# Dizzy-cell/HOUV

Hardware: AMD Instinct MI355X
Metric: registration pairs/sec (2048-pt partial pairs) (higher is better)
Workload: dtype f32; 1 GPU; HOUV solve_model, 2048x2048-pt pairs, batch 256/GPU, K=64 restarts x 200 Adam iterations + retry stages (BASELINE configs[1]); pairs_per_gpu=256, points=2048, kernel=64, iters=200, icp_refine=False, parallelism=dp1 (pair shards, one RCCL all-gather of [steps*P,12] per rank)

## Files before the change

houv_amd/csrc/houv_math.h:

```cpp
#pragma once
#include <math.h>

#if defined(__HIPCC__)
#define HOUV_HD __host__ __device__
#else
#define HOUV_HD
#endif

namespace houv {

constexpr float kPiF = 3.14159274101257324f;

enum TransMode { kTransHouv = 0, kTransSolve = 1 };

HOUV_HD inline float tsqrt(float x) { return sqrtf(x); }
HOUV_HD inline double tsqrt(double x) { return sqrt(x); }

struct Pose {
  float R[9];
  float T[3];
  float u[3], inv_vnorm, sin_t, cos_t, chat[3], inv_cnorm, sigma, a, s;
};

HOUV_HD inline void pose_forward(const float p[8], int angle_base, int trans_mode, Pose& o) {
// ... 34 lines not shown
      AtM[i * 3 + j] = A[0 * 3 + i] * M[0 * 3 + j] + A[1 * 3 + i] * M[1 * 3 + j] + A[2 * 3 + i] * M[2 * 3 + j];
    }
  float dth = 0.f;
  for (int i = 0; i < 9; ++i) dth += M[i] * (f.cos_t * A[i] + f.sin_t * AA[i]);
  g[3] = dth * cosf(f.a * kPiF) * kPiF * kPiF / 8.0f;
  float Qm[9];
  const float omc = 1.0f - f.cos_t;
  for (int i = 0; i < 9; ++i) Qm[i] = f.sin_t * M[i] + omc * (MAt[i] + AtM[i]);
  const float du0 = Qm[7] - Qm[5], du1 = Qm[2] - Qm[6], du2 = Qm[3] - Qm[1];
  const float dot_u = ux * du0 + uy * du1 + uz * du2;
  g[0] = (du0 - ux * dot_u) * f.inv_vnorm;
  g[1] = (du1 - uy * dot_u) * f.inv_vnorm;
  g[2] = (du2 - uz * dot_u) * f.inv_vnorm;
  const float dot_c = f.chat[0] * gT[0] + f.chat[1] * gT[1] + f.chat[2] * gT[2];
  g[4] = f.sigma * (gT[0] - f.chat[0] * dot_c) * f.inv_cnorm;
  g[5] = f.sigma * (gT[1] - f.chat[1] * dot_c) * f.inv_cnorm;
  g[6] = f.sigma * (gT[2] - f.chat[2] * dot_c) * f.inv_cnorm;
  const float dsig = (trans_mode == kTransHouv) ? (cosf(f.s * kPiF) * kPiF * 0.125f) : (cosf(f.s * kPiF) * kPiF);
  g[7] = dot_c * dsig;
}

struct AdamScalars {
  double step_size, bc2_sqrt;
};
HOUV_HD inline AdamScalars adam_scalars(int step, double lr, double b1, double b2) {
  const double bc1 = 1.0 - pow(b1, (double)step);
  const double bc2 = 1.0 - pow(b2, (double)step);
  return AdamScalars{lr / bc1, sqrt(bc2)};
}
template <typename T>
HOUV_HD inline void adam_step(T& p, T& m, T& v, T g, const AdamScalars& sc, double b1, double b2, double eps) {
  m = m + (g - m) * (T)(1.0 - b1);
  v = v * (T)b2 + ((T)(1.0 - b2) * g) * g;
  const T denom = tsqrt(v) / (T)sc.bc2_sqrt + (T)eps;
  p = p - (T)sc.step_size * (m / denom);
}
template <typename T>
HOUV_HD inline void adam_step(T& p, T& m, T& v, T g, int step, double lr, double b1, double b2, double eps) {
  adam_step<T>(p, m, v, g, adam_scalars(step, lr, b1, b2), b1, b2, eps);
}

constexpr int kAccN = 13;
constexpr int kAccStride = 16;

struct TailLoss {
  float score, loss;
  float cd[4][2];
  float g[8];
};

template <int NMET>
HOUV_HD inline void solve_tail_loss(const float* acc, int acc_stride, const Pose& f, int k_full, int k_view, float loss_scale,
                                    int trans_mode, TailLoss& r) {
  float val[NMET];
  int pick[NMET];
  float gT[3] = {0.f, 0.f, 0.f}, Mm[9] = {0.f, 0.f, 0.f, 0.f, 0.f, 0.f, 0.f, 0.f, 0.f};
  bool bad = false;
#pragma unroll
  for (int m = 0; m < 4; ++m) r.cd[m][0] = r.cd[m][1] = 0.f;
#pragma unroll
  for (int m = 0; m < NMET; ++m) {
    const float kk = (float)((m == 0) ? k_full : k_view);
    r.cd[m][0] = acc[(m * 2 + 0) * acc_stride] / kk;
    r.cd[m][1] = acc[(m * 2 + 1) * acc_stride] / kk;
    pick[m] = (r.cd[m][0] <= r.cd[m][1]) ? 0 : 1;
    val[m] = r.cd[m][pick[m]];
    if (r.cd[m][0] != r.cd[m][0] || r.cd[m][1] != r.cd[m][1]) { val[m] = NAN; bad = true; }
    const float w = ((m == 0) ? 6.0f : 1.0f) * loss_scale / kk;
    const float* ac = acc + (m * 2 + pick[m]) * acc_stride;
#pragma unroll
    for (int i = 0; i < 3; ++i) gT[i] += w * ac[1 + i];
#pragma unroll
    for (int i = 0; i < 9; ++i) Mm[i] += w * ac[4 + i];
  }
  r.score = val[0];
  r.loss = val[0] * 6.0f;
  if constexpr (NMET == 4) r.loss = r.loss + (val[1] + val[2] + val[3]);
  if (bad) {
#pragma unroll
    for (int i = 0; i < 3; ++i) gT[i] = NAN;
#pragma unroll
    for (int i = 0; i < 9; ++i) Mm[i] = NAN;
  }
  pose_backward(f, trans_mode, gT, Mm, r.g);
}

HOUV_HD inline void solve_tail_step(const float g[8], double* state, int f64_params, AdamScalars asc, double beta1, double beta2,
                                    double eps, int angle_base, int trans_mode, Pose& next) {
  if (f64_params) {
    for (int k = 0; k < 8; ++k)
      adam_step<double>(state[k], state[8 + k], state[16 + k], (double)g[k], asc, beta1, beta2, eps);
  } else {
    for (int k = 0; k < 8; ++k) {
      float pp = (float)state[k], mm = (float)state[8 + k], vv = (float)state[16 + k];
      adam_step<float>(pp, mm, vv, g[k], asc, beta1, beta2, eps);
      state[k] = pp; state[8 + k] = mm; state[16 + k] = vv;
    }
  }
  float p[8];
#pragma unroll
  for (int k = 0; k < 8; ++k) p[k] = (float)state[k];
  pose_forward(p, angle_base, trans_mode, next);
}

constexpr int kTermAnchorFloats = 20;
constexpr float kTermRel = 1e-3f;
constexpr float kTermAbs = 1e-6f;
constexpr float kTermMoveErr = 1e-6f;

template <int NMET>
HOUV_HD inline unsigned term_masks(const float* anchor, const float* R, const float* T, float radius) {
  float fr = 0.f, ft = 0.f, tn = 0.f, ta = 0.f;
#pragma unroll
  for (int i = 0; i < 9; ++i) {
    const float d = R[i] - anchor[8 + i];
    fr += d * d;
  }
#pragma unroll
  for (int i = 0; i < 3; ++i) {
    const float d = T[i] - anchor[17 + i];
    ft += d * d;
    tn += T[i] * T[i];
    ta += anchor[17 + i] * anchor[17 + i];
  }
  const float delta2 = 2.0f * (sqrtf(fr) * radius + sqrtf(ft));
  const float abs_margin = kTermAbs + kTermMoveErr * (2.0f * radius + sqrtf(tn) + sqrtf(ta));
  unsigned need = ((1u << NMET) - 1u) * 0x11u;
#pragma unroll
  for (int m = 0; m < NMET; ++m) {
    const float c0 = anchor[2 * m], c1 = anchor[2 * m + 1];
    const float slack = delta2 + kTermRel * (fabsf(c0) + fabsf(c1) + delta2) + abs_margin;
    const unsigned drop1 = (c0 + slack < c1) ? (0x10u << m) : 0u;
    const unsigned drop0 = (c1 + slack < c0) ? (1u << m) : 0u;
    need &= ~(drop0 | drop1);
  }
  return need;
}

constexpr float kTermDefectMax = 1e-3f;
constexpr float kTermDefectErr = 1e-6f;

HOUV_HD inline float term_rot_defect(const float* M) {
  float s = 0.f;
#pragma unroll
  for (int i = 0; i < 3; ++i)
#pragma unroll
    for (int j = i; j < 3; ++j) {
      const float g = M[i] * M[j] + M[3 + i] * M[3 + j] + M[6 + i] * M[6 + j] - ((i == j) ? 1.0f : 0.0f);
      s += ((i == j) ? 1.0f : 2.0f) * g * g;
    }
  return sqrtf(s) + kTermDefectErr;
}

HOUV_HD inline void term_travel(const float* Rz, const float* Tz, const float* R, const float* T, float def_now, float radius,
                                float& d, float& tz) {
  float fr = 0.f, ft = 0.f, ta = 0.f;
#pragma unroll
  for (int i = 0; i < 9; ++i) {
    const float e = R[i] - Rz[i];
    fr += e * e;
  }
#pragma unroll
  for (int i = 0; i < 3; ++i) {
    const float e = T[i] - Tz[i];
    ft += e * e;
    ta += Tz[i] * Tz[i];
  }
  const float fro = sqrtf(fr), defect = def_now + term_rot_defect(Rz);
  const float tight = fro * 0.70710683f + 2.0f * defect;
  const bool ok = (fr <= 2.0f) & (defect <= kTermDefectMax) & (tight < fro);
  d = (ok ? tight : fro) * radius + sqrtf(ft);
  tz = sqrtf(ta);
}

template <int NMET>
HOUV_HD inline unsigned term_anchor_masks(const float* cd, const float* fresh, const float* stale, int stride,
                                          unsigned stale_bits, const float* R, const float* T, float radius_in) {
  const float radius = fabsf(radius_in);
  const float def_now = term_rot_defect(R);
  const float tn = sqrtf(T[0] * T[0] + T[1] * T[1] + T[2] * T[2]);
  float d_f, t_f;
  term_travel(fresh, fresh + 9, R, T, def_now, radius, d_f, t_f);
  unsigned need = ((1u << NMET) - 1u) * 0x11u;
#pragma unroll
  for (int m = 0; m < NMET; ++m) {
    float Rs[9], Ts[3], d_s, t_s;
#pragma unroll
    for (int i = 0; i < 9; ++i) Rs[i] = stale[(m * 12 + i) * stride];
#pragma unroll
    for (int i = 0; i < 3; ++i) Ts[i] = stale[(m * 12 + 9 + i) * stride];
    term_travel(Rs, Ts, R, T, def_now, radius, d_s, t_s);
    const bool s0 = (stale_bits >> m) & 1u, s1 = (stale_bits >> (4 + m)) & 1u;
    const float d0 = s0 ? d_s : d_f, d1 = s1 ? d_s : d_f;
    const float t0 = s0 ? t_s : t_f, t1 = s1 ? t_s : t_f;
    const float c0 = cd[2 * m], c1 = cd[2 * m + 1];
    const float dd = d0 + d1;
    const float slack = dd + kTermRel * (fabsf(c0) + fabsf(c1) + dd) + kTermAbs +
                        kTermMoveErr * (2.0f * radius + tn + 0.5f * (t0 + t1));
    const unsigned drop1 = (c0 + slack < c1) ? (0x10u << m) : 0u;
    const unsigned drop0 = (c1 + slack < c0) ? (1u << m) : 0u;
    need &= ~(drop0 | drop1);
  }
  return need;
}

constexpr int kWalkSets[] = {6, 11, 12, 13, 15};
constexpr int kNumWalkSets = (int)(sizeof(kWalkSets) / sizeof(kWalkSets[0]));
constexpr int walk_step_cost(unsigned mset) {
  const int k0 = (int)(mset & 1u), k1 = (int)((mset >> 1) & 1u), k2 = (int)((mset >> 2) & 1u), k3 = (int)((mset >> 3) & 1u);
  return 16 * (2 * (k0 + k1 + k2 + ((k0 | k3) ? 1 : 0)) + 2 * k1 + (k0 + k1 + k2 + k3)) + 5 * (k0 + k1 + k2 + k3);
}
constexpr bool walk_instantiated(unsigned mset) {
  for (int i = 0; i < kNumWalkSets; ++i)
    if ((unsigned)kWalkSets[i] == mset) return true;
  return false;
}
constexpr unsigned walk_variant(unsigned need) {
  unsigned best = 15u;
  for (int i = 0; i < kNumWalkSets; ++i) {
    const unsigned s = (unsigned)kWalkSets[i];
    if ((s & need) == need && walk_step_cost(s) < walk_step_cost(best)) best = s;
  }
  return best;
}
static_assert(walk_instantiated(15u) && walk_variant(15u) == 15u && walk_step_cost(15u) == 16 * 14 + 20, "today's code is a variant");
constexpr unsigned long long walk_variant_table() {
  unsigned long long t = 0ull;
  for (unsigned n = 0; n < 16u; ++n) t |= (unsigned long long)walk_variant(n) << (4 * n);
  return t;
}

HOUV_HD inline float box_med3(float a, float b, float c) {
#if defined(__HIP_DEVICE_COMPILE__)
  return __builtin_amdgcn_fmed3f(a, b, c);
#else
  if (a != a || b != b || c != c) return fminf(fminf(a, b), c);
  return fmaxf(fminf(a, b), fminf(fmaxf(a, b), c));
#endif
}

template <int NMET>
HOUV_HD inline bool box_within_bounds(float dx, float dy, float dz, const float* b, unsigned mset) {
  if constexpr (NMET == 4) {
    const float xx = dx * dx, yy = dy * dy;
    const float s3 = __builtin_fmaf(dy, dy, xx), s1 = __builtin_fmaf(dz, dz, yy), s2 = __builtin_fmaf(dz, dz, xx);
    const float s0 = __builtin_fmaf(dz, dz, s3);
    bool in = false;
    if (mset & 1u) in |= s0 <= b[0];
    if (mset & 2u) in |= s1 <= b[1];
    if (mset & 4u) in |= s2 <= b[2];
    if (mset & 8u) in |= s3 <= b[3];
    return in;
  } else {
    return __builtin_fmaf(dz, dz, __builtin_fmaf(dy, dy, dx * dx)) <= b[0];
  }
}

template <int NMET>
HOUV_HD inline bool box_test_query(const float* q, const float* lo, const float* hi, const float* ub, unsigned mset) {
  return box_within_bounds<NMET>(q[0] - box_med3(q[0], lo[0], hi[0]), q[1] - box_med3(q[1], lo[1], hi[1]),
                                 q[2] - box_med3(q[2], lo[2], hi[2]), ub, mset);
}

HOUV_HD inline float box_group_gap(float glo, float ghi, float lo, float hi) {
  return fmaxf(fmaxf(fminf(lo, hi) - ghi, glo - fmaxf(lo, hi)), 0.0f);
}

template <int NMET>
HOUV_HD inline bool box_test_group(const float* glo, const float* ghi, const float* lo, const float* hi, const float* gub,
                                   unsigned mset) {
  return box_within_bounds<NMET>(box_group_gap(glo[0], ghi[0], lo[0], hi[0]), box_group_gap(glo[1], ghi[1], lo[1], hi[1]),
                                 box_group_gap(glo[2], ghi[2], lo[2], hi[2]), gub, mset);
}

template <typename T>
HOUV_HD inline void svd3x3(const T H[9], T U[9], T S[3], T V[9]) {
  T B[9];
  for (int i = 0; i < 9; ++i) { B[i] = H[i]; V[i] = (i % 4 == 0) ? (T)1 : (T)0; }
  const int P[3] = {0, 0, 1}, Qi[3] = {1, 2, 2};
  for (int sweep = 0; sweep < 12; ++sweep) {
    T off = 0;
    for (int r = 0; r < 3; ++r) {
      const int p = P[r], q = Qi[r];
      const T a = B[0 * 3 + p] * B[0 * 3 + p] + B[1 * 3 + p] * B[1 * 3 + p] + B[2 * 3 + p] * B[2 * 3 + p];
      const T b = B[0 * 3 + q] * B[0 * 3 + q] + B[1 * 3 + q] * B[1 * 3 + q] + B[2 * 3 + q] * B[2 * 3 + q];
      const T g = B[0 * 3 + p] * B[0 * 3 + q] + B[1 * 3 + p] * B[1 * 3 + q] + B[2 * 3 + p] * B[2 * 3 + q];
      const T eps2 = sizeof(T) == 4 ? (T)1e-14 : (T)1e-31;
      if (g * g <= eps2 * a * b) continue;
      off += (T)1;
      const T zeta = (b - a) / ((T)2 * g);
      const T az = zeta < 0 ? -zeta : zeta;
      const T t = (zeta < 0 ? (T)-1 : (T)1) / (az + tsqrt((T)1 + zeta * zeta));
      const T c = (T)1 / tsqrt((T)1 + t * t);
      const T s = c * t;
      for (int i = 0; i < 3; ++i) {
        const T bp = B[i * 3 + p], bq = B[i * 3 + q];
        B[i * 3 + p] = c * bp - s * bq;
        B[i * 3 + q] = s * bp + c * bq;
        const T vp = V[i * 3 + p], vq = V[i * 3 + q];
        V[i * 3 + p] = c * vp - s * vq;
        V[i * 3 + q] = s * vp + c * vq;
      }
    }
    if (off == (T)0) break;
  }
  for (int j = 0; j < 3; ++j)
    S[j] = tsqrt(B[0 * 3 + j] * B[0 * 3 + j] + B[1 * 3 + j] * B[1 * 3 + j] + B[2 * 3 + j] * B[2 * 3 + j]);
  auto swapcol = [&](int x, int y) {
    T ts = S[x]; S[x] = S[y]; S[y] = ts;
    for (int i = 0; i < 3; ++i) {
      T tb = B[i * 3 + x]; B[i * 3 + x] = B[i * 3 + y]; B[i * 3 + y] = tb;
      T tv = V[i * 3 + x]; V[i * 3 + x] = V[i * 3 + y]; V[i * 3 + y] = tv;
    }
  };
  if (S[0] < S[1]) swapcol(0, 1);
  if (S[1] < S[2]) swapcol(1, 2);
  if (S[0] < S[1]) swapcol(0, 1);
  const T tiny = S[0] * (sizeof(T) == 4 ? (T)1e-6 : (T)1e-13);
  for (int j = 0; j < 2; ++j) {
    if (S[j] > tiny && S[j] > (T)0) {
      for (int i = 0; i < 3; ++i) U[i * 3 + j] = B[i * 3 + j] / S[j];
    } else if (j == 0) {
      U[0] = 1; U[3] = 0; U[6] = 0;
    } else {
      const T x = U[0], y = U[3], z = U[6];
      const T ax = x < 0 ? -x : x, ay = y < 0 ? -y : y, az = z < 0 ? -z : z;
      T e[3] = {0, 0, 0};
      if (ax <= ay && ax <= az) e[0] = 1; else if (ay <= az) e[1] = 1; else e[2] = 1;
      T w[3] = {y * e[2] - z * e[1], z * e[0] - x * e[2], x * e[1] - y * e[0]};
      const T n = tsqrt(w[0] * w[0] + w[1] * w[1] + w[2] * w[2]);
      U[1] = w[0] / n; U[4] = w[1] / n; U[7] = w[2] / n;
    }
  }
  if (S[2] > tiny && S[2] > (T)0) {
    for (int i = 0; i < 3; ++i) U[i * 3 + 2] = B[i * 3 + 2] / S[2];
  } else {
    U[2] = U[3] * U[7] - U[6] * U[4];
    U[5] = U[6] * U[1] - U[0] * U[7];
    U[8] = U[0] * U[4] - U[3] * U[1];
  }
}

template <typename T>
HOUV_HD inline T det3(const T m[9]) {
  return m[0] * (m[4] * m[8] - m[5] * m[7]) - m[1] * (m[3] * m[8] - m[5] * m[6]) + m[2] * (m[3] * m[7] - m[4] * m[6]);
}

template <typename T>
HOUV_HD inline void kabsch_rotation(const T H[9], T R[9]) {
  T U[9], S[3], V[9];
  svd3x3<T>(H, U, S, V);
  for (int i = 0; i < 3; ++i)
    for (int j = 0; j < 3; ++j) R[i * 3 + j] = V[i * 3 + 0] * U[j * 3 + 0] + V[i * 3 + 1] * U[j * 3 + 1] + V[i * 3 + 2] * U[j * 3 + 2];
  if (det3<T>(R) < (T)0) {
    for (int i = 0; i < 3; ++i)
      for (int j = 0; j < 3; ++j) R[i * 3 + j] = V[i * 3 + 0] * U[j * 3 + 0] + V[i * 3 + 1] * U[j * 3 + 1] - V[i * 3 + 2] * U[j * 3 + 2];
// ... 5 lines not shown
```

houv_amd/csrc/solve.hip:

```cpp
#include <stddef.h>
#include <stdlib.h>

#include "../../include/houv_hip.h"
#include "houv_common.h"
#include "houv_solve.h"

namespace houv {
namespace {

struct SolveArgs : SolveCommon {
  short* nn_ws;
  int ws_valid;
  int ws_stride;
  int pred_mode;
  unsigned long long* stats;
  unsigned long long* walk_hist;
  unsigned long long* cull_stats;
};

constexpr int kRescanBatch = 4;
constexpr int kRefresh = 4;
constexpr int kTermMaxAge = 0;

struct Smem {
  float4* tgt;
  float4* mov;
  double* state;
  double* adam;
  float* pose;
  float* acc;
  float* red;
  unsigned* hist;
  int* ctl;
  float4* tbox;
  float4* mbox;
  SortedStage st;
  float* anchor;
};
constexpr int kAnchorFloats = kTermAnchorFloats + 4;
constexpr int kTermAges = 8;
constexpr int kStalePose = 4;


__host__ __device__ inline int pad_unit(int prune) { return prune == 3 ? 2 * kSub : kSub; }

__host__ __device__ inline size_t smem_bytes(int N, int M, int block, int prune, int q) {
  const int pu = pad_unit(prune);
  int npad = (N + pu - 1) / pu * pu, mpad = (M + pu - 1) / pu * pu;
  if (prune) npad = mpad = (npad > mpad ? npad : mpad);
  const int nw = block / 64;
  const size_t nq = (size_t)block * q;
  return (size_t)(npad + mpad) * 16 + 28 * 8 + kPoseFloats * 4 + 8 * kAccStride * 4 + (size_t)2 * nw * kRedStride * 4 +
         kHistSets * kHistBins * 4 + (8 + nw) * 4 + 64 + (prune ? 2 * 128 * 16 + nq * 2 + 132 * 4 + kAnchorFloats * 4 : 0);
}

__device__ inline Smem carve(unsigned char* base, int N, int M, int block, int nq, int pu) {
  int npad = (N + pu - 1) / pu * pu, mpad = (M + pu - 1) / pu * pu;
  if (nq) npad = mpad = (npad > mpad ? npad : mpad);
  const int nw = block / 64;
  Smem s;
  s.tgt = reinterpret_cast<float4*>(base);
  s.mov = s.tgt + mpad;
  s.state = reinterpret_cast<double*>(s.mov + npad);
  s.adam = s.state + 24;
  s.pose = reinterpret_cast<float*>(s.adam + 4);
  s.acc = s.pose + kPoseFloats;
  s.red = s.acc + 8 * kAccStride;
  s.hist = reinterpret_cast<unsigned*>(s.red + 2 * nw * kRedStride);
  s.ctl = reinterpret_cast<int*>(s.hist + kHistSets * kHistBins);
  const size_t box_off = ((size_t)(reinterpret_cast<unsigned char*>(s.ctl + 8 + nw) - base) + 15) & ~(size_t)15;
  s.tbox = reinterpret_cast<float4*>(base + box_off);
  s.mbox = s.tbox + 128;
  s.st.hist = reinterpret_cast<int*>(s.mbox + 128);
  s.st.order = reinterpret_cast<unsigned short*>(s.st.hist + 132);
  s.anchor = reinterpret_cast<float*>(s.st.order + nq);
  return s;
}

template <typename T>
__device__ __forceinline__ T fresh(T v) {
  asm volatile("" : "+s"(v));
  return v;
}
__device__ __forceinline__ const float* fresh_lds(const float* p) {
  typedef const float __attribute__((address_space(3))) * lds_f;
  return (const float*)(lds_f)(size_t)fresh((unsigned)(size_t)(lds_f)p);
}

template <int BLOCK, int Q>
__device__ __forceinline__ void select_smallest(const unsigned (&key)[Q], int ksel, unsigned* hist, int* ctl,
                                                bool (&sel)[Q], int& hrot) {
  constexpr int NW = BLOCK / 64;
  const int tid = tid_x(), lane = tid & 63, wave = tid >> 6;
  RadixState rs{0u, 0u, ksel, 0};
#pragma unroll
  for (int pass = 0; pass < 4; ++pass) {
    unsigned* h = radix_rotate<BLOCK>(hist, hrot, tid);
#pragma unroll
    for (int k = 0; k < Q; ++k) radix_count(h, key[k], pass, lane, rs);
    __syncthreads();
    radix_pick(h, pass, lane, rs);
  }
  const unsigned prefix = rs.prefix;
  const int remaining = rs.remaining, neq = rs.neq;
  if (neq == remaining) {
#pragma unroll
    for (int k = 0; k < Q; ++k) sel[k] = key[k] <= prefix;
  } else {
    int e = 0;
#pragma unroll
    for (int k = 0; k < Q; ++k) e += (key[k] == prefix) ? 1 : 0;
    const int incl = wave_incl_scan_dpp(e);
    __syncthreads();
    if (lane == 63) ctl[8 + wave] = incl;
    __syncthreads();
    int rank = incl - e;
    for (int w = 0; w < NW; ++w) rank += (w < wave) ? ctl[8 + w] : 0;
#pragma unroll
    for (int k = 0; k < Q; ++k) {
      const bool eq = key[k] == prefix;
      sel[k] = key[k] < prefix || (eq && rank < remaining);
      rank += eq ? 1 : 0;
    }
  }
}

constexpr int kGradN = 12;

__device__ __forceinline__ void park(float v, float* dst) {
  v = wave_sum_to_lane63(v);
  if ((tid_x() & 63) == 63) *dst = v;
}

template <int BLOCK, int Q, int NMET>
__device__ __forceinline__ void select_all(const Smem& sm, const float (&best)[Q][NMET], int count, int k_full, int k_view,
                                           unsigned need, int& hrot, unsigned (&bits)[NMET]) {
  bool valid[Q], sel[Q];
  unsigned key[Q];
#pragma unroll
  for (int m = 0; m < NMET; ++m) {
    const int ksel = (m == 0) ? k_full : k_view;
#pragma unroll
    for (int k = 0; k < Q; ++k) {
      valid[k] = pt_index<BLOCK>(k) < count;
      key[k] = valid[k] ? __float_as_uint(best[k][m]) : 0xFFFFFFFFu;
      sel[k] = valid[k];
    }
    if (ksel < count && ((need >> m) & 1u)) select_smallest<BLOCK, Q>(key, ksel, sm.hist, sm.ctl, sel, hrot);
    unsigned b = 0u;
#pragma unroll
    for (int k = 0; k < Q; ++k) b |= sel[k] ? (1u << k) : 0u;
    bits[m] = b;
  }
}

template <int Q>
__device__ __forceinline__ float lane_sqrt_sum(const float (&bd)[Q], unsigned selbits) {
  float s = 0.f;
#pragma unroll
  for (int k = 0; k < Q; ++k)
    if ((selbits >> k) & 1u) s += (bd[k] < INFINITY) ? sqrtf(bd[k]) : NAN;
  return s;
}

template <int BLOCK, int Q, int MET, int DIR, bool WS>
__device__ __forceinline__ void lane_grad_sums(const Smem& sm, const float4* __restrict__ refs, const float (&qx)[Q],
                                               const float (&qy)[Q], const float (&qz)[Q], const float (&bd)[Q],
                                               const int (&bt)[Q], unsigned selbits, int count, const float (&px)[Q],
                                               const float (&py)[Q], const float (&pz)[Q], float (&g)[kGradN], buf_t ws,
                                               int ws_off) {
  const int rot = tid_x() & (kSub - 1);
#pragma unroll
  for (int i = 0; i < kGradN; ++i) g[i] = 0.f;
  float R[9], T[3];
  if constexpr (DIR == 0) load_rt(sm.pose, R, T);
#pragma unroll
  for (int k = 0; k < Q; ++k) {
    int jn;
    const float4 nn = recover_nn<MET, kRescanBatch, true>(refs + bt[k] * kTrk, qx[k], qy[k], qz[k], bd[k], rot, jn);
    if (WS && pt_index<BLOCK>(k) < count)
      __builtin_amdgcn_raw_buffer_store_b16((unsigned short)(bt[k] * kTrk + jn), ws, tid_x() * kNnRec,
                                            ws_off + pt_base<BLOCK>(k) * kNnRec + MET * 2, 0);
    if ((selbits >> k) & 1u) {
      const float s = (bd[k] < INFINITY) ? sqrtf(bd[k]) : NAN;
      const float inv = 1.0f / s;
      float dx, dy, dz, sx, sy, sz;
      if constexpr (DIR == 1) {
        dx = qx[k] - nn.x; dy = qy[k] - nn.y; dz = qz[k] - nn.z;
        sx = px[k]; sy = py[k]; sz = pz[k];
      } else {
        dx = nn.x - qx[k]; dy = nn.y - qy[k]; dz = nn.z - qz[k];
        const float ux = nn.x - T[0], uy = nn.y - T[1], uz = nn.z - T[2];
        sx = R[0] * ux + R[3] * uy + R[6] * uz;
        sy = R[1] * ux + R[4] * uy + R[7] * uz;
        sz = R[2] * ux + R[5] * uy + R[8] * uz;
      }
      if constexpr (MET == 1) dx = 0.f;
      if constexpr (MET == 2) dy = 0.f;
      if constexpr (MET == 3) dz = 0.f;
      const float cx = dx * inv, cy = dy * inv, cz = dz * inv;
      g[0] += cx; g[1] += cy; g[2] += cz;
      g[3] += cx * sx; g[4] += cx * sy; g[5] += cx * sz;
      g[6] += cy * sx; g[7] += cy * sy; g[8] += cy * sz;
      g[9] += cz * sx; g[10] += cz * sy; g[11] += cz * sz;
    }
  }
}

template <int BLOCK, int Q, int NMET>
__device__ __forceinline__ void park_sqrt_sums(const float (&best)[Q][NMET], const unsigned (&selbits)[NMET], unsigned need,
                                               float* red_wave) {
  float bd[Q];
#pragma unroll
  for (int m = 0; m < NMET; ++m) {
    if (!((need >> m) & 1u)) continue;
#pragma unroll
    for (int k = 0; k < Q; ++k) bd[k] = best[k][m];
    park(lane_sqrt_sum<Q>(bd, selbits[m]), red_wave + m * kAccN);
  }
}

template <int BLOCK, int Q, int NMET, int DIR, bool WS>
__device__ __forceinline__ void park_grad_sums(const Smem& sm, const float4* __restrict__ refs, const float (&qx)[Q],
                                               const float (&qy)[Q], const float (&qz)[Q], const float (&best)[Q][NMET],
                                               const int (&btile)[Q][NMET], const unsigned (&selbits)[NMET], unsigned mask,
                                               int count, const float (&px)[Q], const float (&py)[Q], const float (&pz)[Q],
                                               float* red_wave, buf_t ws, int ws_off) {
  float bd[Q], g[kGradN];
  int bt[Q];
#define HOUV_GRAD(MET)                                                                                              \
  if ((mask >> MET) & 1u) {                                                                                         \
    _Pragma("unroll") for (int k = 0; k < Q; ++k) {                                                                 \
      bd[k] = best[k][MET];                                                                                         \
      bt[k] = btile[k][MET];                                                                                        \
    }                                                                                                               \
    lane_grad_sums<BLOCK, Q, MET, DIR, WS>(sm, refs, qx, qy, qz, bd, bt, selbits[MET], count, px, py, pz, g,        \
                                           ws, ws_off);                                                             \
    _Pragma("unroll") for (int i = 0; i < kGradN; ++i) park(g[i], red_wave + MET * kAccN + 1 + i);                  \
  }
  HOUV_GRAD(0)
  if constexpr (NMET == 4) {
    HOUV_GRAD(1)
    HOUV_GRAD(2)
    HOUV_GRAD(3)
  }
#undef HOUV_GRAD
}

template <int BLOCK, int NMET>
__device__ __forceinline__ void final_sums(const Smem& sm, int dir, bool want_s, unsigned grad_mask, unsigned need) {
  constexpr int NW = BLOCK / 64;
  const int tid = tid_x();
  if (tid < NMET * kAccN) {
    const int m = tid / kAccN, i = tid % kAccN;
    if ((i == 0) ? want_s : (((grad_mask >> m) & 1u) != 0u)) {
      const float* r = sm.red + (size_t)dir * NW * kRedStride + tid;
      float a = 0.f;
#pragma unroll
      for (int w = 0; w < NW; ++w) a += r[w * kRedStride];
      if (i == 0 && !((need >> m) & 1u)) a = INFINITY;
      sm.acc[(m * 2 + dir) * kAccStride + i] = a;
    }
  }
}

template <int NMET>
__device__ __forceinline__ unsigned picked_direction(const Smem& sm, int k_full, int k_view) {
  unsigned pick = 0u;
#pragma unroll
  for (int m = 0; m < NMET; ++m) {
    const float kk = (float)((m == 0) ? k_full : k_view);
    const float cd0 = sm.acc[(m * 2 + 0) * kAccStride] / kk, cd1 = sm.acc[(m * 2 + 1) * kAccStride] / kk;
    pick |= (cd0 <= cd1) ? 0u : (1u << m);
  }
  return pick;
}

template <int BLOCK>
__device__ __forceinline__ void load_src_point(buf_t src, int k, int N, float& x, float& y, float& z) {
  x = y = z = 0.f;
  if (pt_index<BLOCK>(k) < N) {
    const auto v = __builtin_amdgcn_raw_buffer_load_b96(src, tid_x() * 12, pt_base<BLOCK>(k) * 12, 0);
    x = __uint_as_float(v[0]); y = __uint_as_float(v[1]); z = __uint_as_float(v[2]);
  }
}

template <int BLOCK, int Q, int MET>
__device__ __forceinline__ void repair_direction_a(const Smem& sm, buf_t src, int N, int mpad, int k_sel,
                                                   int& hrot, float* red_wave) {
  float sx[Q], sy[Q], sz[Q], mx[Q], my[Q], mz[Q];
  float R[9], T[3];
  load_rt(sm.pose, R, T);
#pragma unroll
  for (int k = 0; k < Q; ++k) {
    load_src_point<BLOCK>(src, k, N, sx[k], sy[k], sz[k]);
    move_point(R, T, sx[k], sy[k], sz[k], mx[k], my[k], mz[k]);
  }
  float bd[Q];
  int bt[Q];
  sweep_one<Q, MET>(sm.tgt, mpad / kTrk, mx, my, mz, bd, bt);
  bool sel[Q];
  unsigned key[Q], bits = 0u;
#pragma unroll
  for (int k = 0; k < Q; ++k) {
    sel[k] = pt_index<BLOCK>(k) < N;
    key[k] = sel[k] ? __float_as_uint(bd[k]) : 0xFFFFFFFFu;
  }
  if (k_sel < N) select_smallest<BLOCK, Q>(key, k_sel, sm.hist, sm.ctl, sel, hrot);
#pragma unroll
  for (int k = 0; k < Q; ++k) bits |= sel[k] ? (1u << k) : 0u;
  float g[kGradN];
  lane_grad_sums<BLOCK, Q, MET, 1, false>(sm, sm.tgt, mx, my, mz, bd, bt, bits, N, sx, sy, sz, g, src, 0);
#pragma unroll
  for (int i = 0; i < kGradN; ++i) park(g[i], red_wave + MET * kAccN + 1 + i);
}

template <int BLOCK, int Q, int NMET, int PRUNE>
__global__ __launch_bounds__(BLOCK, (Q == 1 ? 8 : 4)) void solve_kernel(SolveArgs a) {
  static_assert(PRUNE == 0 || PRUNE == 2 || PRUNE == 3, "brute force, or the balanced walk over sub-tiles / super-tiles");
  constexpr int TS = (PRUNE == 3) ? 1 : 0;
  constexpr int kPad = kSub << TS;
  extern __shared__ __attribute__((aligned(512))) unsigned char smem_raw[];
  const int N = a.N, M = a.M;
  const Smem sm = carve(smem_raw, N, M, BLOCK, PRUNE ? BLOCK * Q : 0, kPad);
  const int tid = tid_x();
  const int ninst = a.P * a.K;
  int inst = blockIdx.x;
  if ((ninst & 7) == 0) inst = (blockIdx.x & 7) * (ninst >> 3) + (blockIdx.x >> 3);
  const int pair = inst / a.K;
  const buf_t src = make_buf(a.src + (size_t)pair * N * 3, N * 12);
  const float* __restrict__ tgt = a.tgt + (size_t)pair * M * 3;
  const int npad = (N + kPad - 1) / kPad * kPad, mpad = (M + kPad - 1) / kPad * kPad;
  const float4 pad4 = make_float4(INFINITY, INFINITY, INFINITY, 0.f);

  for (int j = tid; j < mpad; j += BLOCK) sm.tgt[j] = (j < M) ? make_float4(tgt[j * 3], tgt[j * 3 + 1], tgt[j * 3 + 2], 0.f) : pad4;
  for (int j = N + tid; j < npad; j += BLOCK) sm.mov[j] = pad4;
  if (tid < 24) sm.state[tid] = a.state[(size_t)inst * 24 + tid];
  for (int j = tid; j < kHistBins; j += BLOCK) sm.hist[j] = 0u;
  if constexpr (PRUNE) {
    if (tid < 132) sm.st.hist[tid] = 0;
  }
  int hrot = 0;
  __syncthreads();
  buf_t ws = src;
  const int ws_b = 0, ws_a = a.ws_stride * kNnRec;
  float4* ws_res = nullptr;
  if constexpr (PRUNE) {
    ws = make_buf(a.nn_ws + (size_t)inst * 16 * a.ws_stride, 32 * a.ws_stride);
    ws_res = reinterpret_cast<float4*>(a.nn_ws + ((size_t)inst * 16 + 8) * a.ws_stride);
    float tx0[Q], ty0[Q], tz0[Q];
#pragma unroll
    for (int k = 0; k < Q; ++k) {
      const int i = pt_index<BLOCK>(k);
      const float4 v = (i < M) ? sm.tgt[i] : make_float4(0.f, 0.f, 0.f, 0.f);
      tx0[k] = v.x; ty0[k] = v.y; tz0[k] = v.z;
    }
    tile_boxes<BLOCK, Q, TS>(tx0, ty0, tz0, M, mpad / kPad, sm.tbox);
  }
  constexpr int kAdamTid = BLOCK >= 128 ? 64 : 0;
  if (tid == 0) {
    float p[8];
#pragma unroll
    for (int k = 0; k < 8; ++k) p[k] = (float)sm.state[k];
    Pose f;
    pose_forward(p, a.angle_base, a.trans_mode, f);
    store_pose(sm.pose, f);
  }
  if (tid == kAdamTid) {
    const int step = a.steps_done + 1;
    const AdamScalars asc = adam_scalars(step, a.lr, a.beta1, a.beta2);
    sm.adam[(step & 1) * 2 + 0] = asc.step_size;
    sm.adam[(step & 1) * 2 + 1] = asc.bc2_sqrt;
  }
  if constexpr (PRUNE) {
    float r2 = 0.f;
#pragma unroll
    for (int k = 0; k < Q; ++k) {
      float x, y, z;
      load_src_point<BLOCK>(src, k, N, x, y, z);
      const float v = __builtin_fmaf(z, z, __builtin_fmaf(y, y, x * x));
      r2 = (v <= r2) ? r2 : ((v < INFINITY) ? v : INFINITY);
    }
#pragma unroll
    for (int o = 1; o < 64; o <<= 1) r2 = fmaxf(r2, __shfl_xor(r2, o, 64));
    if ((tid & 63) == 0) sm.red[tid >> 6] = r2;
    if (tid == 0) {
      sm.ctl[0] = (int)(((1u << NMET) - 1u) * 0x11u);
      reinterpret_cast<unsigned*>(sm.anchor)[kTermAges] = 0u;
    }
  }
  __syncthreads();
  if constexpr (PRUNE) {
    if (tid == 0) {
      float r2 = 0.f;
      for (int w = 0; w < BLOCK / 64; ++w) r2 = fmaxf(r2, sm.red[w]);
      sm.anchor[kTermAnchorFloats] = sqrtf(r2) * 1.000001f;
    }
  }

  unsigned long long clk0 = 0ull, rt0 = 0ull;
  if (a.stats) {
    clk0 = __builtin_amdgcn_s_memtime();
    rt0 = __builtin_amdgcn_s_memrealtime();
  }
  constexpr int NW = BLOCK / 64;
  constexpr unsigned kAllMet = (1u << NMET) - 1u;
  unsigned pred_a = kAllMet;
  auto red_row = [&](int dir) { return sm.red + ((size_t)dir * NW + (tid_x() >> 6)) * kRedStride; };
#pragma unroll 1
  for (int it = 0; it < a.n_iters; ++it) {
    if (a.pred_mode == 1) pred_a = 0u;
    const bool allgrad = a.pred_mode == 2 || ((PRUNE != 0) && (((a.steps_done + it) % kRefresh) == 0 || (a.ws_valid == 0 && it == 0)));
    unsigned need_a = kAllMet, need_b = kAllMet;
    if constexpr (PRUNE != 0) {
      const unsigned w = (unsigned)__builtin_amdgcn_readfirstlane(*reinterpret_cast<const int*>(fresh_lds(reinterpret_cast<const float*>(sm.ctl))));
      need_b = w & kAllMet;
      need_a = (w >> 4) & kAllMet;
    }
    const unsigned grad_a = (allgrad ? kAllMet : (pred_a | ~need_b)) & need_a;
    {
      float sx[Q], sy[Q], sz[Q], mx[Q], my[Q], mz[Q];
      float R[9], T[3];
      load_rt(fresh_lds(sm.pose), R, T);
#pragma unroll
      for (int k = 0; k < Q; ++k) {
        const int i = pt_index<BLOCK>(k);
        const bool ok = i < N;
        load_src_point<BLOCK>(src, k, N, sx[k], sy[k], sz[k]);
        move_point(R, T, sx[k], sy[k], sz[k], mx[k], my[k], mz[k]);
        if (ok) sm.mov[i] = make_float4(mx[k], my[k], mz[k], 0.f);
      }
      __syncthreads();
      bool pruned_now = false;
      float best[Q][NMET];
      int btile[Q][NMET];
      if constexpr (PRUNE) {
        tile_boxes<BLOCK, Q, TS>(mx, my, mz, N, npad / kPad, sm.mbox);
        pruned_now = (a.ws_valid != 0) || (it > 0);
      }
      if (need_a != 0u) {
        if (pruned_now) {
          if constexpr (PRUNE != 0)
            pruned_sweep_sorted<BLOCK, Q, NMET, TS>(sm.tgt, sm.tbox, mpad / kPad, sm.mbox, sm.mov, sm.tgt, sm.mov, mx, my, mz, ws, ws_a, N,
                                                need_a, sm.st, ws_res, best, btile, a.stats, fresh(a.walk_hist), fresh(a.cull_stats));
        } else {
          sweep<Q, NMET>(sm.tgt, mpad / kTrk, mx, my, mz, best, btile);
          if (a.stats && (tid & 63) == 0) atomicAdd(&a.stats[3], 1ull);
        }
        unsigned sel[NMET];
        select_all<BLOCK, Q, NMET>(sm, best, N, a.k_full, a.k_view, need_a, hrot, sel);
        park_sqrt_sums<BLOCK, Q, NMET>(best, sel, need_a, red_row(1));
        park_grad_sums<BLOCK, Q, NMET, 1, PRUNE != 0>(sm, sm.tgt, mx, my, mz, best, btile, sel, grad_a, N, sx, sy, sz, red_row(1), ws,
                                                     ws_a);
      }
      __syncthreads();
      final_sums<BLOCK, NMET>(sm, 1, true, grad_a, need_a);
    }
    unsigned pick_a;
    {
      float tx[Q], ty[Q], tz[Q];
#pragma unroll
      for (int k = 0; k < Q; ++k) {
        const int i = pt_index<BLOCK>(k);
        const float4 v = (i < M) ? sm.tgt[i] : make_float4(0.f, 0.f, 0.f, 0.f);
        tx[k] = v.x; ty[k] = v.y; tz[k] = v.z;
      }
      const bool pruned_now = (PRUNE != 0) && ((a.ws_valid != 0) || (it > 0));
      auto pick_winners = [&]() {
        __syncthreads();
        final_sums<BLOCK, NMET>(sm, 0, true, 0u, need_b);
        __syncthreads();
        pick_a = picked_direction<NMET>(sm, fresh(a.k_full), fresh(a.k_view));
        return (allgrad ? kAllMet : (~pick_a & kAllMet)) & need_b;
      };
      unsigned grad_b = 0u;
      if (need_b != 0u) {
        float best[Q][NMET];
        int btile[Q][NMET];
        if (pruned_now) {
          if constexpr (PRUNE != 0)
            pruned_sweep_sorted<BLOCK, Q, NMET, TS>(sm.mov, sm.mbox, npad / kPad, sm.tbox, sm.tgt, sm.tgt, sm.mov, tx, ty, tz, ws, ws_b, M,
                                                need_b, sm.st, ws_res, best, btile, a.stats, fresh(a.walk_hist), fresh(a.cull_stats));
        } else {
          sweep<Q, NMET>(sm.mov, npad / kTrk, tx, ty, tz, best, btile);
          if (a.stats && (tid & 63) == 0) atomicAdd(&a.stats[3], 1ull);
        }
        unsigned sel[NMET];
        select_all<BLOCK, Q, NMET>(sm, best, M, a.k_full, a.k_view, need_b, hrot, sel);
        park_sqrt_sums<BLOCK, Q, NMET>(best, sel, need_b, red_row(0));
        grad_b = pick_winners();
        park_grad_sums<BLOCK, Q, NMET, 0, PRUNE != 0>(sm, sm.mov, tx, ty, tz, best, btile, sel, grad_b, M, tx, ty, tz, red_row(0), ws,
                                                     ws_b);
      } else {
        pick_winners();
      }
      const unsigned miss = pick_a & ~grad_a & kAllMet;
      if (miss) {
        if (miss & 1u) repair_direction_a<BLOCK, Q, 0>(sm, src, N, mpad, a.k_full, hrot, red_row(1));
        if constexpr (NMET == 4) {
          if (miss & 2u) repair_direction_a<BLOCK, Q, 1>(sm, src, N, mpad, a.k_view, hrot, red_row(1));
          if (miss & 4u) repair_direction_a<BLOCK, Q, 2>(sm, src, N, mpad, a.k_view, hrot, red_row(1));
          if (miss & 8u) repair_direction_a<BLOCK, Q, 3>(sm, src, N, mpad, a.k_view, hrot, red_row(1));
        }
      }
      __syncthreads();
      final_sums<BLOCK, NMET>(sm, 0, false, grad_b, kAllMet);
      if (miss) final_sums<BLOCK, NMET>(sm, 1, false, miss, kAllMet);
    }
    pred_a = pick_a;
    static_assert(NMET * kAccN <= 64, "final_sums runs on the scalar tail's wave");
    __builtin_amdgcn_wave_barrier();

    if (kAdamTid != 0 && tid == kAdamTid && it + 1 < a.n_iters) {
      const int step = a.steps_done + it + 2;
      const AdamScalars asc = adam_scalars(step, fresh(a.lr), fresh(a.beta1), fresh(a.beta2));
      sm.adam[(step & 1) * 2 + 0] = asc.step_size;
      sm.adam[(step & 1) * 2 + 1] = asc.bc2_sqrt;
    }
    if (tid == 0) {
      const int k_full = fresh(a.k_full), k_view = fresh(a.k_view);
      const float loss_scale = fresh(a.loss_scale);
      const double lr = fresh(a.lr), beta1 = fresh(a.beta1), beta2 = fresh(a.beta2), eps = fresh(a.eps);
      const int angle_base = fresh(a.angle_base), trans_mode = fresh(a.trans_mode);
      Pose f;
      load_pose(f, sm.pose);
      TailLoss r;
      solve_tail_loss<NMET>(sm.acc, kAccStride, f, k_full, k_view, loss_scale, trans_mode, r);
      if (it == a.n_iters - 1)
        store_outputs(a.out_score, a.out_loss, a.out_R, a.out_T, a.out_grad, a.out_cd, inst, f, r);
      if constexpr (PRUNE != 0) {
#pragma unroll
        for (int m = 0; m < NMET; ++m) {
          if ((need_b >> m) & 1u) sm.anchor[2 * m] = r.cd[m][0];
          if ((need_a >> m) & 1u) sm.anchor[2 * m + 1] = r.cd[m][1];
        }
      }
      const int step = a.steps_done + it + 1;
      const AdamScalars asc{sm.adam[(step & 1) * 2 + 0], sm.adam[(step & 1) * 2 + 1]};
      solve_tail_step(r.g, sm.state, a.f64_params, asc, beta1, beta2, eps, angle_base, trans_mode, f);
      if constexpr (PRUNE != 0) {
        unsigned next = kAllMet | (kAllMet << 4), ages = 0u;
        const bool all_next = fresh(a.pred_mode) == 2 || it + 2 >= a.n_iters;
        if (!all_next) {
          const unsigned have = need_b | (need_a << 4);
          float* stale = reinterpret_cast<float*>(sm.tbox) + 3;
          next = term_anchor_masks<NMET>(sm.anchor, sm.pose, stale, kStalePose, ~have & 0xffu, f.R, f.T,
                                         sm.anchor[kTermAnchorFloats]);
          const unsigned old_ages = reinterpret_cast<const unsigned*>(sm.anchor)[kTermAges];
#pragma unroll
          for (int m = 0; m < NMET; ++m) {
            unsigned age = (old_ages >> (8 * m)) & 0xffu;
            age = (((next >> m) & (next >> (4 + m)) & 1u) != 0u) ? 0u : age + 1u;
            if (kTermMaxAge > 0 && age > (unsigned)kTermMaxAge) {
              next |= 0x11u << m;
              age = 0u;
            }
            if (age > 0xffu) age = 0xffu;
            ages |= age << (8 * m);
            if (((have & ~next) >> m) & 0x11u) {
#pragma unroll
              for (int i = 0; i < 12; ++i) stale[(m * 12 + i) * kStalePose] = sm.pose[i];
            }
          }
        }
        reinterpret_cast<unsigned*>(sm.anchor)[kTermAges] = ages;
        sm.ctl[0] = (int)next;
        if (a.stats) {
          atomicAdd(&a.stats[6], (unsigned long long)(__popc(need_a) + __popc(need_b)));
          atomicAdd(&a.stats[7], (unsigned long long)(2 * NMET));
        }
      }
      store_pose(sm.pose, f);
      if (kAdamTid == 0 && it + 1 < a.n_iters) {
        const AdamScalars nxt = adam_scalars(step + 1, lr, beta1, beta2);
        sm.adam[((step + 1) & 1) * 2 + 0] = nxt.step_size;
        sm.adam[((step + 1) & 1) * 2 + 1] = nxt.bc2_sqrt;
      }
    }
    __syncthreads();
  }
  if (tid_x() < 24) a.state[(size_t)inst * 24 + tid_x()] = sm.state[tid_x()];
  if (a.stats) {
    const unsigned long long dc = __builtin_amdgcn_s_memtime() - clk0, dr = __builtin_amdgcn_s_memrealtime() - rt0;
    if (tid == 0) {
      atomicAdd(&a.stats[4], dc);
      atomicAdd(&a.stats[5], dr);
    }
  }
}

template <int BLOCK, int Q, int PRUNE>
int launch(const SolveArgs& a, int use_views, hipStream_t s) {
  const size_t bytes = smem_bytes(a.N, a.M, BLOCK, PRUNE, Q);
  const int grid = a.P * a.K;
  hipError_t e;
  if (use_views) {
    e = hipFuncSetAttribute((const void*)solve_kernel<BLOCK, Q, 4, PRUNE>, hipFuncAttributeMaxDynamicSharedMemorySize, (int)bytes);
    if (e != hipSuccess) { set_error("houv_solve_iterate: cannot reserve %zu B of LDS: %s", bytes, hipGetErrorString(e)); return 0; }
    solve_kernel<BLOCK, Q, 4, PRUNE><<<grid, BLOCK, bytes, s>>>(a);
  } else {
    e = hipFuncSetAttribute((const void*)solve_kernel<BLOCK, Q, 1, PRUNE>, hipFuncAttributeMaxDynamicSharedMemorySize, (int)bytes);
    if (e != hipSuccess) { set_error("houv_solve_iterate: cannot reserve %zu B of LDS: %s", bytes, hipGetErrorString(e)); return 0; }
    solve_kernel<BLOCK, Q, 1, PRUNE><<<grid, BLOCK, bytes, s>>>(a);
  }
  return check_launch("houv_solve_iterate") ? 1 : 0;
}

}
}

extern "C" int houv_solve_variant(int N, int M, int pruned, int* block, int* points_per_lane, int* prune_mode) {
  using namespace houv;
  const int mx = N > M ? N : M;
  if (N <= 0 || M <= 0) {
    set_error("houv_solve_variant: bad cloud sizes N=%d M=%d", N, M);
    return 0;
  }
  if (mx > 4096) {
    set_error("houv_solve_iterate: clouds larger than 4096 points do not fit in 160 KiB of LDS (N=%d M=%d)", N, M);
    return 0;
  }
  int b, q;
  if (mx <= 64) { b = 64; q = 1; }
  else if (mx <= 128) { b = 128; q = 1; }
  else if (mx <= 256) { b = 256; q = 1; }
  else if (mx <= 512) { b = 256; q = 2; }
  else if (mx <= 768) { b = 256; q = 3; }
  else if (mx <= 1024) { b = 256; q = 4; }
  else if (mx <= 1536) { b = 512; q = 3; }
  else if (mx <= 2048) { b = 512; q = 4; }
  else if (mx <= 3072) { b = 1024; q = 3; }
  else { b = 1024; q = 4; }
  if (block) *block = b;
  if (points_per_lane) *points_per_lane = q;
  constexpr int kPrunedMinPoints = 257;
  if (prune_mode) *prune_mode = (!pruned || mx < kPrunedMinPoints) ? 0 : (mx > 2048) ? 3 : 2;
  return 1;
}

extern "C" int houv_solve_walk_variant(int need) {
  if (need < 0 || need > 15) {
    houv::set_error("houv_solve_walk_variant: the term mask of a direction is 0..15, got %d", need);
    return -1;
  }
  return (int)houv::walk_variant((unsigned)need);
}

extern "C" long long houv_solve_lds_bytes(int N, int M, int pruned) {
  using namespace houv;
  int block = 0, q = 0, mode = 0;
  if (!houv_solve_variant(N, M, pruned, &block, &q, &mode)) return -1;
  return (long long)smem_bytes(N, M, block, mode, q);
}

int houv::solve_check_args(const char* who, const SolveCommon& a, int use_views) {
  const int P = a.P, N = a.N, M = a.M;
  if (P < 0 || N <= 0 || M <= 0 || a.K <= 0 || a.n_iters <= 0 || a.steps_done < 0 || a.angle_base < 0 || a.angle_base > 3 ||
      a.trans_mode < 0 || a.trans_mode > 1) {
    set_error("%s: bad argument P=%d N=%d M=%d K=%d n_iters=%d steps_done=%d base=%d trans_mode=%d", who, P, N, M, a.K,
              a.n_iters, a.steps_done, a.angle_base, a.trans_mode);
    return 0;
  }
  if (P == 0) return 1;
  if (!a.src || !a.tgt || !a.state) {
    set_error("%s: null pointer", who);
    return 0;
  }
  const int kv = use_views ? a.k_view : 1;
  if (a.k_full < 1 || a.k_full > N || a.k_full > M || kv < 1 || kv > N || kv > M) {
    set_error("%s: top-k size out of range (k_full=%d k_view=%d N=%d M=%d)", who, a.k_full, a.k_view, N, M);
    return 0;
  }
  if ((long long)P * a.K > 0x7fffffffLL) {
    set_error("%s: too many hypotheses", who);
    return 0;
  }
  return 2;
}

static int solve_dispatch(const houv::SolveCommon& c, int use_views, short* nn_ws, int ws_valid, int ws_stride, bool prune,
                          void* stream, const char* who) {
  using namespace houv;
  const int ok = solve_check_args(who, c, use_views);
  if (ok < 2) return ok;
  const int N = c.N, M = c.M;
  SolveArgs a{c, nn_ws, ws_valid, ws_stride, g_debug.pred_mode.load(),
              reinterpret_cast<unsigned long long*>(g_debug.stats.load()),
              reinterpret_cast<unsigned long long*>(g_debug.walk_hist.load()),
              reinterpret_cast<unsigned long long*>(g_debug.cull_stats.load())};
  hipStream_t s = (hipStream_t)stream;
  const int mx = N > M ? N : M;
  int block = 0, q = 0, mode = 0;
  if (!houv_solve_variant(N, M, prune ? 1 : 0, &block, &q, &mode)) return 0;
  if (prune && (!nn_ws || ws_stride < mx || (ws_stride & 7))) {
    set_error("%s: pruned mode needs a workspace of 16 x ws_stride int16 per hypothesis, ws_stride >= max(N,M) and a multiple of 8", who);
    return 0;
  }
  if (prune && ((uintptr_t)nn_ws & 15)) {
    set_error("%s: the pruned-mode workspace must be 16-byte aligned", who);
    return 0;
// ... 44 lines not shown
```

Measured before the change: 215.8 pairs/s.

## Tighten metric-skip travel bound using source cloud centre and radii

Computes the source cloud's bounding-box centre, its max distance from that centre and its mean distance once per block. The termination/anchor test that decides which chamfer metrics can be skipped on the next iteration now bounds pose travel through the centred displacement, using mean radius where all points contribute. The tighter bound should let more metric evaluations be skipped. In exchange it adds a second reduction pass and a barrier at setup, plus extra per-iteration arithmetic in the mask logic.

```diff
diff --git a/houv_amd/csrc/houv_math.h b/houv_amd/csrc/houv_math.h
--- a/houv_amd/csrc/houv_math.h
+++ b/houv_amd/csrc/houv_math.h
@@ -210,47 +210,88 @@
   return sqrtf(s) + kTermDefectErr;
 }
 
-HOUV_HD inline void term_travel(const float* Rz, const float* Tz, const float* R, const float* T, float def_now, float radius,
-                                float& d, float& tz) {
-  float fr = 0.f, ft = 0.f, ta = 0.f;
+constexpr int kTermCloudFloats = 6;
+constexpr float kTermUErr = 1e-6f;
+constexpr float kTermSumInfl = 1.0003f;
+constexpr float kTermSumAbs = 1e-18f;
+HOUV_HD inline float term_cloud_dist2(float x, float y, float z, const float* c) {
+  const float dx = x - c[0], dy = y - c[1], dz = z - c[2];
+  return dz * dz + (dy * dy + dx * dx);
+}
+HOUV_HD inline float term_cloud_mean(float sum, int n) { return sum / (float)n * kTermSumInfl + kTermSumAbs; }
+
+struct TermTravel {
+  float d;
+  float tz;
+  float rho;
+  float un;
+};
+
+template <bool CENTRED>
+HOUV_HD inline TermTravel term_travel(const float* Rz, const float* Tz, const float* R, const float* T, float def_now, float tn,
+                                      float radius, const float* c) {
+  float fr = 0.f, ft = 0.f, ta = 0.f, uu = 0.f, cc = 0.f;
+  float e[9], t[3];
 #pragma unroll
   for (int i = 0; i < 9; ++i) {
-    const float e = R[i] - Rz[i];
-    fr += e * e;
+    e[i] = R[i] - Rz[i];
+    fr += e[i] * e[i];
   }
 #pragma unroll
   for (int i = 0; i < 3; ++i) {
-    const float e = T[i] - Tz[i];
-    ft += e * e;
+    t[i] = T[i] - Tz[i];
+    ft += t[i] * t[i];
     ta += Tz[i] * Tz[i];
   }
   const float fro = sqrtf(fr), defect = def_now + term_rot_defect(Rz);
   const float tight = fro * 0.70710683f + 2.0f * defect;
   const bool ok = (fr <= 2.0f) & (defect <= kTermDefectMax) & (tight < fro);
-  d = (ok ? tight : fro) * radius + sqrtf(ft);
-  tz = sqrtf(ta);
-}
-
-template <int NMET>
-HOUV_HD inline unsigned term_anchor_masks(const float* cd, const float* fresh, const float* stale, int stride,
-                                          unsigned stale_bits, const float* R, const float* T, float radius_in) {
+  TermTravel r;
+  r.rho = ok ? tight : fro;
+  r.d = r.rho * radius + sqrtf(ft);
+  r.tz = sqrtf(ta);
+  r.un = 0.f;
+  if (CENTRED) {
+#pragma unroll
+    for (int i = 0; i < 3; ++i) {
+      const float ui = e[3 * i + 2] * c[2] + (e[3 * i + 1] * c[1] + (e[3 * i] * c[0] + t[i]));
+      uu += ui * ui;
+      cc += c[i] * c[i];
+    }
+    r.un = sqrtf(uu) + kTermUErr * (fro * sqrtf(cc) + tn + r.tz);
+  }
+  return r;
+}
+
+template <bool CENTRED>
+HOUV_HD inline float term_travel_pick(const TermTravel& v, float rad) {
+  if (!CENTRED) return v.d;
+  const float d_new = v.rho * rad + v.un;
+  return (d_new < v.d) ? d_new : v.d + 0.0f * d_new;
+}
+
+template <int NMET, bool CENTRED>
+HOUV_HD inline unsigned term_record_masks(const float* cd, const float* fresh, const float* stale, int stride,
+                                          unsigned stale_bits, const float* R, const float* T, float radius_in,
+                                          const float* cloud) {
   const float radius = fabsf(radius_in);
+  const float r_max = CENTRED ? fabsf(cloud[3]) : 0.f, r_view = CENTRED ? fabsf(cloud[4]) : 0.f, r_top = CENTRED ? fabsf(cloud[5]) : 0.f;
   const float def_now = term_rot_defect(R);
   const float tn = sqrtf(T[0] * T[0] + T[1] * T[1] + T[2] * T[2]);
-  float d_f, t_f;
-  term_travel(fresh, fresh + 9, R, T, def_now, radius, d_f, t_f);
+  const TermTravel f = term_travel<CENTRED>(fresh, fresh + 9, R, T, def_now, tn, radius, cloud);
   unsigned need = ((1u << NMET) - 1u) * 0x11u;
 #pragma unroll
   for (int m = 0; m < NMET; ++m) {
-    float Rs[9], Ts[3], d_s, t_s;
+    float Rs[9], Ts[3];
 #pragma unroll
     for (int i = 0; i < 9; ++i) Rs[i] = stale[(m * 12 + i) * stride];
 #pragma unroll
     for (int i = 0; i < 3; ++i) Ts[i] = stale[(m * 12 + 9 + i) * stride];
-    term_travel(Rs, Ts, R, T, def_now, radius, d_s, t_s);
+    const TermTravel s = term_travel<CENTRED>(Rs, Ts, R, T, def_now, tn, radius, cloud);
     const bool s0 = (stale_bits >> m) & 1u, s1 = (stale_bits >> (4 + m)) & 1u;
-    const float d0 = s0 ? d_s : d_f, d1 = s1 ? d_s : d_f;
-    const float t0 = s0 ? t_s : t_f, t1 = s1 ? t_s : t_f;
+    const float rad1 = (m == 0) ? r_top : r_view;
+    const float d0 = term_travel_pick<CENTRED>(s0 ? s : f, r_max), d1 = term_travel_pick<CENTRED>(s1 ? s : f, rad1);
+    const float t0 = s0 ? s.tz : f.tz, t1 = s1 ? s.tz : f.tz;
     const float c0 = cd[2 * m], c1 = cd[2 * m + 1];
     const float dd = d0 + d1;
     const float slack = dd + kTermRel * (fabsf(c0) + fabsf(c1) + dd) + kTermAbs +
@@ -260,6 +301,18 @@
     need &= ~(drop0 | drop1);
   }
   return need;
+}
+
+template <int NMET>
+HOUV_HD inline unsigned term_anchor_masks(const float* cd, const float* fresh, const float* stale, int stride,
+                                          unsigned stale_bits, const float* R, const float* T, float radius) {
+  return term_record_masks<NMET, false>(cd, fresh, stale, stride, stale_bits, R, T, radius, nullptr);
+}
+
+template <int NMET>
+HOUV_HD inline unsigned term_travel_masks(const float* cd, const float* fresh, const float* stale, int stride,
+                                          unsigned stale_bits, const float* R, const float* T, float radius, const float* cloud) {
+  return term_record_masks<NMET, true>(cd, fresh, stale, stride, stale_bits, R, T, radius, cloud);
 }
 
 constexpr int kWalkSets[] = {6, 11, 12, 13, 15};
diff --git a/houv_amd/csrc/solve.hip b/houv_amd/csrc/solve.hip
--- a/houv_amd/csrc/solve.hip
+++ b/houv_amd/csrc/solve.hip
@@ -38,6 +38,8 @@
   float* anchor;
 };
 constexpr int kAnchorFloats = kTermAnchorFloats + 4;
+constexpr int kTermCloud = 9;
+static_assert(kTermCloud + kTermCloudFloats <= kTermAnchorFloats, "the cloud's scalars live in the free floats of the anchor block");
 constexpr int kTermAges = 8;
 constexpr int kStalePose = 4;
 
@@ -315,6 +317,20 @@
   for (int i = 0; i < kGradN; ++i) park(g[i], red_wave + MET * kAccN + 1 + i);
 }
 
+template <int BLOCK>
+__device__ __forceinline__ void cloud_centre(const float* red, float (&c)[3]) {
+  float l0 = INFINITY, l1 = INFINITY, l2 = INFINITY, h0 = -INFINITY, h1 = -INFINITY, h2 = -INFINITY;
+#pragma unroll 1
+  for (int w = 0; w < BLOCK / 64; ++w) {
+    const float* row = red + w * kRedStride;
+    l0 = fminf(l0, row[1]); l1 = fminf(l1, row[2]); l2 = fminf(l2, row[3]);
+    h0 = fmaxf(h0, row[4]); h1 = fmaxf(h1, row[5]); h2 = fmaxf(h2, row[6]);
+  }
+  c[0] = 0.5f * l0 + 0.5f * h0;
+  c[1] = 0.5f * l1 + 0.5f * h1;
+  c[2] = 0.5f * l2 + 0.5f * h2;
+}
+
 template <int BLOCK, int Q, int NMET, int PRUNE>
 __global__ __launch_bounds__(BLOCK, (Q == 1 ? 8 : 4)) void solve_kernel(SolveArgs a) {
   static_assert(PRUNE == 0 || PRUNE == 2 || PRUNE == 3, "brute force, or the balanced walk over sub-tiles / super-tiles");
@@ -373,28 +389,85 @@
     sm.adam[(step & 1) * 2 + 1] = asc.bc2_sqrt;
   }
   if constexpr (PRUNE) {
-    float r2 = 0.f;
+    float r2 = 0.f, lo[3] = {INFINITY, INFINITY, INFINITY}, hi[3] = {-INFINITY, -INFINITY, -INFINITY};
+    float px[Q], py[Q], pz[Q];
 #pragma unroll
     for (int k = 0; k < Q; ++k) {
-      float x, y, z;
-      load_src_point<BLOCK>(src, k, N, x, y, z);
-      const float v = __builtin_fmaf(z, z, __builtin_fmaf(y, y, x * x));
+      load_src_point<BLOCK>(src, k, N, px[k], py[k], pz[k]);
+      const float v = __builtin_fmaf(pz[k], pz[k], __builtin_fmaf(py[k], py[k], px[k] * px[k]));
       r2 = (v <= r2) ? r2 : ((v < INFINITY) ? v : INFINITY);
-    }
-#pragma unroll
-    for (int o = 1; o < 64; o <<= 1) r2 = fmaxf(r2, __shfl_xor(r2, o, 64));
-    if ((tid & 63) == 0) sm.red[tid >> 6] = r2;
+      if (pt_index<BLOCK>(k) < N) {
+        lo[0] = fminf(lo[0], px[k]); lo[1] = fminf(lo[1], py[k]); lo[2] = fminf(lo[2], pz[k]);
+        hi[0] = fmaxf(hi[0], px[k]); hi[1] = fmaxf(hi[1], py[k]); hi[2] = fmaxf(hi[2], pz[k]);
+      }
+    }
+#pragma unroll
+    for (int o = 1; o < 64; o <<= 1) {
+      r2 = fmaxf(r2, __shfl_xor(r2, o, 64));
+#pragma unroll
+      for (int i = 0; i < 3; ++i) {
+        lo[i] = fminf(lo[i], __shfl_xor(lo[i], o, 64));
+        hi[i] = fmaxf(hi[i], __shfl_xor(hi[i], o, 64));
+      }
+    }
+    static_assert(kRedStride >= 7, "a wave's row of sm.red holds r2 | lo | hi");
+    if ((tid & 63) == 0) {
+      float* row = sm.red + (tid >> 6) * kRedStride;
+      row[0] = r2;
+#pragma unroll
+      for (int i = 0; i < 3; ++i) {
+        row[1 + i] = lo[i];
+        row[4 + i] = hi[i];
+      }
+    }
     if (tid == 0) {
       sm.ctl[0] = (int)(((1u << NMET) - 1u) * 0x11u);
       reinterpret_cast<unsigned*>(sm.anchor)[kTermAges] = 0u;
     }
+    __syncthreads();
+    float c[3];
+    cloud_centre<BLOCK>(sm.red, c);
+    float q2 = 0.f, qs = 0.f;
+#pragma unroll
+    for (int k = 0; k < Q; ++k) {
+      if (pt_index<BLOCK>(k) < N) {
+        const float v = term_cloud_dist2(px[k], py[k], pz[k], c);
+        q2 = (v <= q2) ? q2 : ((v < INFINITY) ? v : INFINITY);
+        qs += (v < INFINITY) ? sqrtf(v) : INFINITY;
+      }
+    }
+#pragma unroll
+    for (int o = 1; o < 64; o <<= 1) {
+      q2 = fmaxf(q2, __shfl_xor(q2, o, 64));
+      qs += __shfl_xor(qs, o, 64);
+    }
+    if ((tid & 63) == 0) {
+      float* row = sm.red + (BLOCK / 64 + (tid >> 6)) * kRedStride;
+      row[0] = q2;
+      row[1] = qs;
+    }
   }
   __syncthreads();
   if constexpr (PRUNE) {
     if (tid == 0) {
-      float r2 = 0.f;
-      for (int w = 0; w < BLOCK / 64; ++w) r2 = fmaxf(r2, sm.red[w]);
+      float r2 = 0.f, q2 = 0.f, qs = 0.f, c[3];
+#pragma unroll 1
+      for (int w = 0; w < BLOCK / 64; ++w) {
+        r2 = fmaxf(r2, sm.red[w * kRedStride]);
+        q2 = fmaxf(q2, sm.red[(BLOCK / 64 + w) * kRedStride]);
+        qs += sm.red[(BLOCK / 64 + w) * kRedStride + 1];
+      }
+      cloud_centre<BLOCK>(sm.red, c);
+      const bool finite = r2 < INFINITY;
+      const float r_max = finite ? sqrtf(q2) * 1.000001f : INFINITY;
+      const float r_mean = finite ? term_cloud_mean(qs, N) : INFINITY;
       sm.anchor[kTermAnchorFloats] = sqrtf(r2) * 1.000001f;
+      float* cloud = sm.anchor + kTermCloud;
+#pragma unroll
+      for (int i = 0; i < 3; ++i) cloud[i] = c[i];
+      cloud[3] = r_max;
+      cloud[4] = (a.k_view >= N) ? r_mean : r_max;
+      cloud[5] = (a.k_full >= N) ? r_mean : r_max;
     }
   }
 
@@ -544,8 +617,8 @@
         if (!all_next) {
           const unsigned have = need_b | (need_a << 4);
           float* stale = reinterpret_cast<float*>(sm.tbox) + 3;
-          next = term_anchor_masks<NMET>(sm.anchor, sm.pose, stale, kStalePose, ~have & 0xffu, f.R, f.T,
-                                         sm.anchor[kTermAnchorFloats]);
+          next = term_travel_masks<NMET>(sm.anchor, sm.pose, stale, kStalePose, ~have & 0xffu, f.R, f.T,
+                                         sm.anchor[kTermAnchorFloats], sm.anchor + kTermCloud);
           const unsigned old_ages = reinterpret_cast<const unsigned*>(sm.anchor)[kTermAges];
 #pragma unroll
           for (int m = 0; m < NMET; ++m) {
```

Result: no change. 217.0 pairs/s (median of 6 runs) (+0.5%).
